# Adamtaranto/mimeo

Measured on AMD Instinct MI355X. Metric: Gbp-aligned/sec (mimeo self, 1 Gbp genome, --minIdt 80 --minLen 100 --minCov 3), higher is better.
Workload: dtype int32

## Files before the change

mimeo_amd/csrc/k6.h:

```cpp
#pragma once
#include <algorithm>
#include <cstdio>
#include <cstdlib>
#include <vector>

#include "device_util.h"

namespace mimeo {

constexpr int32_t NEG = -(1 << 30);
constexpr int32_t NEGH = -(1 << 29);

struct Cell {
    int32_t s;
    uint32_t nm, nx;
};
struct HalfResult {
    int32_t score;
    uint32_t i, j, nm, nx, overflow;
    uint32_t maxcols, rows;
    uint32_t base_lo, base_hi;
};
struct DpJob {
    uint32_t group, at, aq;
// ... 130 lines not shown
        }
        nt = dir > 0 ? min(nt, c) : max(nt, c);
    }
    for (int o = 32; o > 0; o >>= 1) {
        kmin = max(kmin, __shfl_xor(kmin, o));
        kmax = min(kmax, __shfl_xor(kmax, o));
        const long long on = __shfl_xor(nt, o);
        nt = dir > 0 ? min(nt, on) : max(nt, on);
    }
    RowBound r;
    r.kmin = wave_uniform_ll(kmin); r.kmax = wave_uniform_ll(kmax);
    nt = wave_uniform_ll(nt);
    const long long nrow = dir > 0 ? nt - (long long)at + 1 : (long long)at - nt;
    r.next = nrow > 0xFFFFFFFEll ? 0xFFFFFFFFu : (uint32_t)nrow;
    r.any = (r.kmin > -K_INF || r.kmax < K_INF) ? 1u : 0u;
    return r;
}
__device__ __forceinline__ bool bounds_none(const BoundCtx &B, uint64_t b0, uint32_t nacc, uint32_t at, int dir) {
    bool hit = false;
    for (uint32_t e = threadIdx.x & 63u; e < nacc; e += 64u) {
        const mimeo_alignment o = B.aln[b0 + e];
        if (o.tend > o.tstart && (dir > 0 ? o.tend > at : o.tstart < at)) hit = true;
    }
    return __ballot(hit) == 0;
}

struct K6Buffers {
    DeviceBuf anchors, packed, jobs, res, cnt, astate, ovf_list, any;
    DeviceBuf pidx, accrank, arena, pool, tjobs, tres, tctr;
    DeviceBuf kjobs, pcnt, pslot, ptmp;
    DeviceBuf sweep;
};
extern K6Buffers g_k6;
int dp_round(Group *d_groups, uint32_t n, const mimeo_params *p, int32_t cap, bool bounded, const BoundCtx &bc, unsigned int *novf);
int arena_reserve(uint64_t blocks, uint64_t used);
struct TraceStats { uint64_t arena_used, largest; float ms; uint32_t slices; };
int trace_round(Group *d_groups, const DpJob *d_jobs, uint32_t h0, const mimeo_params *p, int32_t cap, uint64_t budget, TraceStats &ts, bool bounded, BoundCtx bc);
int paths_pass(Group *d_groups, uint32_t ngroups, const mimeo_params *p, int32_t cap, const mimeo_alignment *d_aln, uint64_t budget, bool k6_stats);

}
```

mimeo_amd/csrc/k6_dp.hip:

```cpp
#include "k6_band.h"

namespace mimeo {

template <int WSTRIP>
__device__ __forceinline__ void load_qbits(const GStrandView &Q, uint32_t aq, int dir, uint32_t jb, uint32_t lenB,
                                           uint32_t &qlo, uint32_t &qhi, uint32_t &qn) {
    constexpr uint32_t SMASK = WSTRIP == 32 ? 0xFFFFFFFFu : ((1u << (WSTRIP & 31)) - 1u);
    if (jb > lenB) { qlo = qhi = qn = 0; return; }
    if (dir > 0) {
        int32_t p = (int32_t)(aq + jb) - 1;
        const Win32 w = win32(Q, p);
        qlo = w.lo & SMASK; qhi = w.hi & SMASK; qn = w.nm & SMASK;
    } else {
        int32_t p = (int32_t)aq - (int32_t)jb - (WSTRIP - 1);
        const Win32 w = win32(Q, p);
        qlo = __brev(w.lo & SMASK) >> (32 - WSTRIP); qhi = __brev(w.hi & SMASK) >> (32 - WSTRIP);
        qn = __brev(w.nm & SMASK) >> (32 - WSTRIP);
    }
}

struct RowBases { uint32_t lo, hi, nm; };
__device__ __forceinline__ RowBases load_row_bases(const GStrandView &T, uint32_t at, int dir, uint32_t i0) {
    if (dir > 0) {
        const Win32 w = win32(T, (int32_t)(at + i0 - 1u));
// ... 110 lines not shown
        if (rl == 63u) { best.overflow = 1; break; }
        best.maxcols = max(best.maxcols, (rl + 1u) * WSTRIP);
        best.rows = i;
        if (__ballot(rb.s > best.score)) {
            const Best4 t = wave_best(rb);
            if (t.s > best.score) { best.score = t.s; best.i = i; best.j = t.j; best.nm = t.nm; best.nx = t.nx; }
            if (best.score > cap) { best.overflow = 1; break; }
        }
        const uint32_t fmask = (uint32_t)__builtin_amdgcn_readlane((int)amask, (int)rf);
        const uint32_t plo = wb + rf * WSTRIP + (uint32_t)__builtin_ctz(fmask);
        const uint32_t nwb = plo & ~(uint32_t)(WSTRIP - 1);
        if (nwb != wb) {
            const uint32_t shift = (nwb - wb) / WSTRIP;
            wb = nwb;
            jb = wb + lane * WSTRIP;
            const int src = (int)((lane + shift) & 63u);
            const bool fresh = lane + shift >= 64u;
#pragma unroll
            for (int s = 0; s < WSTRIP; s++) {
                int32_t cs = __shfl(Cs[s], src), ds = __shfl(Ds[s], src);
                Cm[s] = __shfl(Cm[s], src); Cx[s] = __shfl(Cx[s], src);
                Dm[s] = __shfl(Dm[s], src); Dx[s] = __shfl(Dx[s], src);
                Cs[s] = fresh ? NEG : cs;
                Ds[s] = fresh ? NEG : ds;
            }
            uint32_t a0 = __shfl(qlo, src), a1 = __shfl(qhi, src), a2 = __shfl(qn, src);
            if (fresh) load_qbits<WSTRIP>(Q, aq, dir, jb, lenB, qlo, qhi, qn);
            else { qlo = a0; qhi = a1; qn = a2; }
        }
    }
    return best;
}

constexpr int L_WS = 14, L_WINDOW = 64 * L_WS;
struct LeanState {
    int32_t C[L_WS], D[L_WS];
    uint32_t Cc[L_WS], Dc[L_WS], sel[L_WS];
};
struct PCell {
    int32_t s;
    uint32_t c;
};
__device__ __forceinline__ PCell pcmax_left(const PCell &l, const PCell &r) { return r.s > l.s ? r : l; }
template <int CTRL, int RMASK>
__device__ __forceinline__ PCell dpp_pcell(const PCell &c) {
    PCell o;
    o.s = __builtin_amdgcn_update_dpp(NEG, c.s, CTRL, RMASK, 0xf, false);
    o.c = (uint32_t)__builtin_amdgcn_update_dpp(0, (int)c.c, CTRL, RMASK, 0xf, false);
    return o;
}

__device__ __forceinline__ int32_t wave_max_i32(int32_t v) {
    v = max(v, __builtin_amdgcn_update_dpp(INT32_MIN, v, 0x111, 0xf, 0xf, false));
    v = max(v, __builtin_amdgcn_update_dpp(INT32_MIN, v, 0x112, 0xf, 0xf, false));
    v = max(v, __builtin_amdgcn_update_dpp(INT32_MIN, v, 0x114, 0xf, 0xf, false));
    v = max(v, __builtin_amdgcn_update_dpp(INT32_MIN, v, 0x118, 0xf, 0xf, false));
    v = max(v, __builtin_amdgcn_update_dpp(INT32_MIN, v, 0x142, 0xa, 0xf, false));
    v = max(v, __builtin_amdgcn_update_dpp(INT32_MIN, v, 0x143, 0xc, 0xf, false));
    return __builtin_amdgcn_readlane(v, 63);
}

template <int CTRL, int RMASK>
__device__ __forceinline__ PCell lean_scan_step(const PCell &v) {
    PCell o;
    o.s = __builtin_amdgcn_update_dpp(v.s, v.s, CTRL, RMASK, 0xf, false);
    o.c = (uint32_t)__builtin_amdgcn_update_dpp((int)v.c, (int)v.c, CTRL, RMASK, 0xf, false);
    return pcmax_left(o, v);
}
__device__ __forceinline__ PCell lean_incl_maxscan(PCell v) {
    v = lean_scan_step<0x111, 0xf>(v);
    v = lean_scan_step<0x112, 0xf>(v);
    v = lean_scan_step<0x114, 0xf>(v);
    v = lean_scan_step<0x118, 0xf>(v);
    v = lean_scan_step<0x142, 0xa>(v);
    v = lean_scan_step<0x143, 0xc>(v);
    return v;
}

__device__ __forceinline__ void lean_selectors(LeanState &S, uint32_t qlo, uint32_t qhi, uint32_t qn) {
#pragma unroll
    for (int s = 0; s < L_WS; s++) {
        const uint32_t idx = ((qlo >> s) & 1u) | (((qhi >> s) & 1u) << 1);
        S.sel[s] = 0x0C0C0C00u | (((qn >> s) & 1u) ? 4u : idx);
    }
}

template <bool EDGE, bool BND = false>
__device__ __forceinline__ int32_t lean_row(LeanState &S, uint32_t srow, int32_t O, int32_t E, int32_t thr, uint32_t exmask,
                                            int32_t lane_base, int32_t kneg128) {
    const int32_t OE = O + E;
    PCell pc = dpp_pcell<0x138, 0xf>(PCell{S.C[L_WS - 1], S.Cc[L_WS - 1]});
#pragma unroll
    for (int s = L_WS - 1; s >= 0; s--) {
        const int32_t t1 = S.D[s] - E, t2 = S.C[s] - OE;
        const bool open = t2 > t1;
        const int32_t ds = max(t1, t2);
        const uint32_t dc = open ? S.Cc[s] : S.Dc[s];
        const PCell left = s ? PCell{S.C[s ? s - 1 : 0], S.Cc[s ? s - 1 : 0]} : pc;
        const uint32_t scb = __builtin_amdgcn_perm(28u, srow, S.sel[s]);
        const int32_t gs = left.s + (int32_t)scb + kneg128;
        const uint32_t gc = left.c + 0x10000u + ((int32_t)scb > 128 ? 1u : 0u);
        const bool vert = ds > gs;
        S.D[s] = ds; S.Dc[s] = dc;
        S.C[s] = max(gs, ds);
        if (BND) S.C[s] = ((exmask >> s) & 1u) ? S.C[s] : NEG;
        S.Cc[s] = vert ? dc : gc;
    }
    PCell run{NEG, 0};
#pragma unroll
    for (int s = 0; s < L_WS; s++) {
        const bool take = S.C[s] > run.s;
        run.c = take ? S.Cc[s] : run.c;
        run.s = max(run.s, S.C[s]) - E;
    }
    run.s += lane_base;
    PCell acc = dpp_pcell<0x138, 0xf>(lean_incl_maxscan(run));
    acc.s += L_WS * E - lane_base;
    int32_t rowmax = NEG;
#pragma unroll
    for (int s = 0; s < L_WS; s++) {
        const int32_t hs = S.C[s];
        const uint32_t hc = S.Cc[s];
        const int32_t is = acc.s - O;
        const bool ins = is > hs;
        const int32_t cs = max(hs, is);
        const uint32_t cc = ins ? acc.c : hc;
        const bool take = hs > acc.s;
        acc.c = take ? hc : acc.c;
        acc.s = max(acc.s, hs) - E;
        bool alive = cs >= thr;
        if (EDGE) alive = alive && ((exmask >> s) & 1u);
        S.C[s] = alive ? cs : NEG; S.Cc[s] = cc;
        S.D[s] = alive ? S.D[s] : NEG;
        rowmax = max(rowmax, S.C[s]);
    }
    return rowmax;
}

template <bool BOUND>
__device__ HalfResult wave_half_extend_lean(const GStrandView &T, const GStrandView &Q, uint32_t at, uint32_t aq, int dir,
                                            int32_t O, int32_t E, int32_t Y, const BoundCtx &B, uint64_t b0, uint32_t nacc,
                                            HalfSweep *sw) {
    const uint32_t lane = threadIdx.x & 63u;
    const uint32_t lenA = dir > 0 ? T.len - at : at, lenB = dir > 0 ? Q.len - aq : aq;
    HalfResult best{0, 0, 0, 0, 0, 0, 0, 0};
    if (BOUND) *sw = HalfSweep{0, 0, nacc, 0};
    if ((!BOUND || bounds_none(B, b0, nacc, at, dir)) && identical_suffix(T, Q, at, aq, dir, best)) return best;
    uint32_t tab[4];
#pragma unroll
    for (uint32_t a = 0; a < 4; a++) {
        uint32_t w = 0;
#pragma unroll
        for (uint32_t b = 0; b < 4; b++) {
            const uint32_t alo = a & 1u, ahi = a >> 1, dl = alo ^ (b & 1u), dh = ahi ^ (b >> 1);
            w |= (uint32_t)(sub_score(dl, dh, alo ^ ahi, 0u) + 128) << (8u * b);
        }
        tab[a] = w;
    }
    LeanState S;
    uint32_t wb = 0, jb = lane * L_WS;
    {
        uint32_t qlo, qhi, qn;
        load_qbits<L_WS>(Q, aq, dir, jb, lenB, qlo, qhi, qn);
        lean_selectors(S, qlo, qhi, qn);
    }
    bool over = false;
#pragma unroll
    for (int s = 0; s < L_WS; s++) {
        const uint32_t j = jb + s;
        const int32_t v = j ? -O - (int32_t)j * E : 0;
        const bool alive = j <= lenB && (j == 0 || v >= -Y);
        S.C[s] = alive ? v : NEG; S.Cc[s] = 0;
        S.D[s] = NEG; S.Dc[s] = 0;
        if (alive && j >= (uint32_t)(L_WINDOW - L_WS)) over = true;
    }
    if (__ballot(over)) { best.overflow = 1; return best; }
    const int32_t lane_base = (int32_t)(lane * L_WS) * E;
    const int32_t kneg128 = __builtin_amdgcn_readfirstlane(-128);
    uint32_t exmask = (1u << L_WS) - 1u;
    bool edge = wb + (uint32_t)L_WINDOW - 1u > lenB;
    if (edge) {
        exmask = 0;
#pragma unroll
        for (int s = 0; s < L_WS; s++) exmask |= (jb + s <= lenB ? 1u : 0u) << s;
    }
    long long bkmin = -K_INF, bkmax = K_INF;
    uint32_t bnext = 1u;
    int32_t klo = INT32_MAX, khi = INT32_MIN;
    RowBases rbase{0, 0, 0}, rnext = load_row_bases(T, at, dir, 1u);
    for (uint32_t i = 1; i <= lenA; i++) {
        if (i >= 0xFFFFu) { best.overflow = 1; break; }
        if (BOUND && i == bnext) {
            const RowBound rb = bounds_at(B, b0, nacc, at, aq, dir, i);
            bkmin = rb.kmin; bkmax = rb.kmax; bnext = rb.next;
        }
        const int32_t thr = best.score - Y;
        const uint32_t rbit = (i - 1u) & 31u;
        if (rbit == 0) { rbase = rnext; rnext = load_row_bases(T, at, dir, i + 32u); }
        const uint32_t rlo = (uint32_t)__builtin_amdgcn_readfirstlane((int)rbase.lo), rhi = (uint32_t)__builtin_amdgcn_readfirstlane((int)rbase.hi),
                       rnm = (uint32_t)__builtin_amdgcn_readfirstlane((int)rbase.nm);
        const uint32_t a = ((rlo >> rbit) & 1u) | (((rhi >> rbit) & 1u) << 1);
        uint32_t srow = a & 2u ? (a & 1u ? tab[3] : tab[2]) : (a & 1u ? tab[1] : tab[0]);
        if ((rnm >> rbit) & 1u) srow = 0x1C1C1C1Cu;
        uint32_t bm = 0;
        bool cut = false;
        if (BOUND) {
            const long long jlo = bkmin + (long long)i + 1, jhi = bkmax + (long long)i - 1;
            if (bkmin > -K_INF || bkmax < K_INF) sw->nbound++;
            cut = jlo > (long long)wb || jhi < (long long)wb + (L_WINDOW - 1);
            const long long r0 = jlo - (long long)jb, r1 = jhi - (long long)jb + 1;
            const uint32_t s0 = (uint32_t)min(max(r0, 0ll), (long long)L_WS), s1 = (uint32_t)min(max(r1, 0ll), (long long)L_WS);
            bm = ((1u << s1) - 1u) & ~((1u << s0) - 1u) & exmask;
        }
        const int32_t rowmax = BOUND && cut ? lean_row<true, true>(S, srow, O, E, thr, bm, lane_base, kneg128)
                               : edge ? lean_row<true>(S, srow, O, E, thr, exmask, lane_base, kneg128)
                                      : lean_row<false>(S, srow, O, E, thr, exmask, lane_base, kneg128);
        const uint64_t ball = __ballot(rowmax > NEGH);
        if (!ball) break;
        const uint32_t rf = (uint32_t)__builtin_ctzll(ball), rl = 63u - (uint32_t)__builtin_clzll(ball);
        if (rl == 63u) { best.overflow = 1; break; }
        best.maxcols = max(best.maxcols, (rl + 1u) * L_WS);
        best.rows = i;
        if (BOUND) {
            klo = min(klo, (int32_t)((long long)wb + rf * L_WS - (long long)i));
            khi = max(khi, (int32_t)((long long)wb + (rl + 1u) * L_WS - 1 - (long long)i));
        }
        const int32_t wmax = wave_max_i32(rowmax);
        if (wmax > best.score) {
            const uint32_t L = (uint32_t)__builtin_ctzll(__ballot(rowmax == wmax));
            uint32_t slot = 0, cnt = 0;
#pragma unroll
            for (int s = L_WS - 1; s >= 0; s--) {
                const int32_t v = __builtin_amdgcn_readlane(S.C[s], (int)L);
                if (v == wmax) { slot = (uint32_t)s; cnt = (uint32_t)__builtin_amdgcn_readlane((int)S.Cc[s], (int)L); }
            }
            best.score = wmax; best.i = i; best.j = wb + L * L_WS + slot; best.nm = cnt & 0xFFFFu; best.nx = (cnt >> 16) - (cnt & 0xFFFFu);
        }
        if (rf) {
            wb += rf * L_WS;
            jb = wb + lane * L_WS;
            const int src = (int)((lane + rf) & 63u);
            const bool fresh = lane + rf >= 64u;
#pragma unroll
            for (int s = 0; s < L_WS; s++) {
                const int32_t cs = __shfl(S.C[s], src), ds = __shfl(S.D[s], src);
                S.Cc[s] = __shfl(S.Cc[s], src); S.Dc[s] = __shfl(S.Dc[s], src);
                S.sel[s] = __shfl(S.sel[s], src);
                S.C[s] = fresh ? NEG : cs;
                S.D[s] = fresh ? NEG : ds;
            }
            if (fresh) {
                uint32_t qlo, qhi, qn;
                load_qbits<L_WS>(Q, aq, dir, jb, lenB, qlo, qhi, qn);
                lean_selectors(S, qlo, qhi, qn);
            }
            edge = wb + (uint32_t)L_WINDOW - 1u > lenB;
            if (edge) {
                exmask = 0;
#pragma unroll
                for (int s = 0; s < L_WS; s++) exmask |= (jb + s <= lenB ? 1u : 0u) << s;
            } else if (BOUND) exmask = (1u << L_WS) - 1u;
        }
    }
    if (BOUND) { sw->klo = klo; sw->khi = khi; }
    return best;
}

__global__ __launch_bounds__(64) void k6_dp1(const Group *__restrict__ groups, const DpJob *__restrict__ jobs,
                                             HalfResult *__restrict__ res, int32_t O, int32_t E, int32_t Y) {
    const DpJob job = jobs[blockIdx.x];
    const Group &G = groups[job.group];
    HalfResult r = wave_half_extend_lean<false>(G.T, G.Q, job.at, job.aq, job.dir, O, E, Y, BoundCtx{}, 0, 0, nullptr);
    if (threadIdx.x == 0) res[job.slot] = r;
}

__global__ __launch_bounds__(64) void k6_dp1_bounded(const Group *__restrict__ groups, const DpJob *__restrict__ jobs,
                                                     HalfResult *__restrict__ res, HalfSweep *__restrict__ sweep, int32_t O, int32_t E,
                                                     int32_t Y, BoundCtx B, unsigned int *__restrict__ novf,
                                                     unsigned int *__restrict__ ovf_list) {
    const DpJob job = jobs[blockIdx.x];
    const Group &G = groups[job.group];
    HalfSweep sw;
    HalfResult r = wave_half_extend_lean<true>(G.T, G.Q, job.at, job.aq, job.dir, O, E, Y, B, G.hsp_begin, G.nacc, &sw);
    if (threadIdx.x == 0) {
        res[job.slot] = r;
        sweep[job.slot] = sw;
        if (r.overflow) ovf_list[atomicAdd(novf, 1u)] = blockIdx.x;
    }
}

__global__ __launch_bounds__(64) void k6_dp_wide(const Group *__restrict__ groups, const DpJob *__restrict__ jobs,
                                                 HalfResult *__restrict__ res, int32_t O, int32_t E, int32_t Y,
                                                 unsigned int *__restrict__ novf, unsigned int *__restrict__ ovf_list, int32_t cap,
                                                 int every) {
    const DpJob job = jobs[blockIdx.x];
    if (!every && !res[job.slot].overflow) return;
    const Group &G = groups[job.group];
    HalfResult r = wave_half_extend_2048(G.T, G.Q, job.at, job.aq, job.dir, O, E, Y, cap);
    if (threadIdx.x == 0) {
        res[job.slot] = r;
        if (r.overflow) ovf_list[atomicAdd(novf, 1u)] = blockIdx.x;
    }
}

constexpr uint32_t ANY_COLS = 1u << 16;
constexpr int ANY_THREADS = 1024;
struct AnyRow {
    int32_t *cs, *ds;
    uint32_t *cm, *cx, *dm, *dx;
};
__device__ __forceinline__ AnyRow any_row(uint32_t *base, uint32_t parity) {
    uint32_t *b = base + (size_t)parity * 6u * ANY_COLS;
    return AnyRow{(int32_t *)b, (int32_t *)(b + ANY_COLS), b + 2u * ANY_COLS, b + 3u * ANY_COLS, b + 4u * ANY_COLS, b + 5u * ANY_COLS};
}
constexpr size_t ANY_SLOT_WORDS = 2u * 6u * (size_t)ANY_COLS;

// ... 17 lines not shown
        if (diag) { g.nm = P.cm[(j - 1) & M] + (m ? 1u : 0u); g.nx = P.cx[(j - 1) & M] + (m ? 0u : 1u); }
        N.dm[j & M] = dd.nm; N.dx[j & M] = dd.nx;
        const Cell hh = hd ? dd : g;
        N.cm[j & M] = hh.nm; N.cx[j & M] = hh.nx;
        return hh;
    }
    __device__ __forceinline__ Cell htag(uint32_t j) const { return Cell{0, N.cm[j & M], N.cx[j & M]}; }
    __device__ __forceinline__ Cell c(uint32_t j, const Cell &ht, const Cell &ia, bool ci) const { const Cell ct = ci ? ia : ht; N.cm[j & M] = ct.nm; N.cx[j & M] = ct.nx; return ct; }
};

template <bool BOUND>
__global__ __launch_bounds__(ANY_THREADS) void k6_dp_any(const Group *__restrict__ groups, const DpJob *__restrict__ jobs,
                                                         const unsigned int *__restrict__ list, uint32_t first,
                                                         HalfResult *__restrict__ res, uint32_t *__restrict__ scratch,
                                                         int32_t O, int32_t E, int32_t Y, int32_t cap, BoundCtx B,
                                                         HalfSweep *__restrict__ sweep) {
    const DpJob job = jobs[list[first + blockIdx.x]];
    const Group &G = groups[job.group];
    const uint32_t lenA = job.dir > 0 ? G.T.len - job.at : job.at;
    CountRows rows{scratch + (size_t)blockIdx.x * ANY_SLOT_WORDS};
    HalfSweep sw;
    const HalfResult r = band_dp<ANY_THREADS, BOUND>(rows, G, job, lenA, O, E, Y, cap, B, sw);
    if (threadIdx.x == 0) res[job.slot] = r;
    if (BOUND && threadIdx.x == 0) sweep[job.slot] = sw;
}

__global__ void k6_list_all(uint32_t n, unsigned int *__restrict__ novf, unsigned int *__restrict__ ovf_list) {
    const uint32_t k = blockIdx.x * blockDim.x + threadIdx.x;
    if (k < n) ovf_list[k] = k;
    if (k == 0) *novf = n;
}

int dp_round(Group *d_groups, uint32_t n, const mimeo_params *p, int32_t cap, bool bounded, const BoundCtx &bc,
                    unsigned int *novf) {
    hipStream_t st = stream();
    int rc;
    const Group *groups = d_groups;
    const DpJob *jobs = (const DpJob *)g_k6.jobs.p;
    HalfResult *res = (HalfResult *)g_k6.res.p;
    HalfSweep *sweep = bounded ? (HalfSweep *)g_k6.sweep.p : nullptr;
    unsigned int *list = (unsigned int *)g_k6.ovf_list.p;
    const int32_t O = p->gap_open, E = p->gap_extend, Y = p->ydrop;
    const bool lean_ok = E <= (1 << 16) && O <= (1 << 24) && Y <= (1 << 28);
    if (bounded) {
        if (lean_ok) hipLaunchKernelGGL(k6_dp1_bounded, dim3(n), dim3(64), 0, st, groups, jobs, res, sweep, O, E, Y, bc, novf, list);
        else hipLaunchKernelGGL(k6_list_all, dim3((n + 255) / 256), dim3(256), 0, st, n, novf, list);
    } else {
        if (lean_ok) hipLaunchKernelGGL(k6_dp1, dim3(n), dim3(64), 0, st, groups, jobs, res, O, E, Y);
        hipLaunchKernelGGL(k6_dp_wide, dim3(n), dim3(64), 0, st, groups, jobs, res, O, E, Y, novf, list, cap, lean_ok ? 0 : 1);
    }
    unsigned int nov = 0;
    HIP_TRY(hipMemcpyAsync(&nov, novf, 4, hipMemcpyDeviceToHost, st));
    HIP_TRY(hipStreamSynchronize(st));
    if (!nov) return 0;
    const unsigned int slots = std::min<unsigned int>(nov, 32u);
    if ((rc = g_k6.any.reserve((size_t)slots * ANY_SLOT_WORDS * 4))) return rc;
    const auto any = bounded ? k6_dp_any<true> : k6_dp_any<false>;
    for (unsigned int f = 0; f < nov; f += slots)
        hipLaunchKernelGGL(any, dim3(std::min(slots, nov - f)), dim3(ANY_THREADS), 0, st, groups, jobs, (const unsigned int *)list, f, res,
                           (uint32_t *)g_k6.any.p, O, E, Y, cap, bc, sweep);
    return 0;
}

}
```

mimeo_amd/csrc/k6_gapped.hip:

```cpp
#include "k6.h"

namespace mimeo {

constexpr uint32_t ANCHOR_W = 31, ANCHOR_CHUNK = 4096;
constexpr int ANCHOR_THREADS = 1024;

__device__ void wave_anchor_chunk(const GStrandView &T, const GStrandView &Q, const mimeo_hsp &h, uint32_t chunk,
                                  unsigned long long *packed) {
    const uint32_t lane = threadIdx.x & 63u, nw = h.length - ANCHOR_W + 1;
    const int32_t d = (int32_t)h.tstart - (int32_t)h.qstart;
    const uint32_t w0 = chunk * ANCHOR_CHUNK + lane * (ANCHOR_CHUNK / 64u), w1 = min(nw, w0 + ANCHOR_CHUNK / 64u);
    int32_t bs = INT32_MIN;
    uint32_t bw = 0xFFFFFFFFu;
    if (w0 < w1) {
        int32_t sum = 0;
        bool m;
        for (uint32_t k = 0; k < ANCHOR_W; k++) {
            int32_t pt = (int32_t)(h.tstart + w0 + k);
            sum += pair_score(T, Q, pt, pt - d, &m);
        }
        bs = sum; bw = w0;
        for (uint32_t w = w0 + 1; w < w1; w++) {
            int32_t add = (int32_t)(h.tstart + w + ANCHOR_W - 1), sub = (int32_t)(h.tstart + w - 1);
            sum += pair_score(T, Q, add, add - d, &m) - pair_score(T, Q, sub, sub - d, &m);
// ... 303 lines not shown

__global__ void k6_kept_ranks(Group *__restrict__ groups, uint32_t ngroups, const mimeo_alignment *__restrict__ aln,
                              uint32_t *__restrict__ accrank, const uint2 *__restrict__ pidx, int32_t thresh) {
    const uint32_t g = blockIdx.x * blockDim.x + threadIdx.x;
    if (g >= ngroups) return;
    Group &G = groups[g];
    const uint64_t b0 = G.hsp_begin;
    uint32_t k = 0;
    for (uint32_t e = 0; e < G.nacc; e++) {
        if (aln[b0 + e].score < thresh) continue;
        const uint32_t rank = accrank[b0 + e];
        const uint32_t slot = 2u * (uint32_t)(b0 + rank);
        if (pidx[slot].x == PATH_UNTRACED || pidx[slot + 1].x == PATH_UNTRACED) G.overflow = 1;
        accrank[b0 + k++] = rank;
    }
}

__global__ __launch_bounds__(256) void k6_ungapped_paths(const Group *__restrict__ groups, const mimeo_alignment *__restrict__ aln,
                                                         PathBlock *__restrict__ arena, uint2 *__restrict__ pidx,
                                                         uint32_t *__restrict__ accrank) {
    const Group &G = groups[blockIdx.x];
    const uint64_t b0 = G.hsp_begin;
    for (uint32_t r = threadIdx.x; r < G.nacc; r += 256) {
        const mimeo_alignment a = aln[b0 + r];
        arena[b0 + r] = PathBlock{a.tstart, a.qstart, a.tend - a.tstart};
        pidx[2u * (b0 + r)] = make_uint2((uint32_t)(b0 + r), 1u);
        pidx[2u * (b0 + r) + 1u] = make_uint2(0u, 0u);
        accrank[b0 + r] = r;
    }
}

K6Buffers g_k6;

static int round_stats(uint32_t n, uint64_t nhsps, bool bounded, unsigned long long *bound_jobs) {
    std::vector<DpJob> hj(n);
    std::vector<HalfResult> hall((size_t)nhsps * 2), hr(n);
    HIP_TRY(hipStreamSynchronize(stream()));
    HIP_TRY(hipMemcpy(hj.data(), g_k6.jobs.p, (size_t)n * sizeof(DpJob), hipMemcpyDeviceToHost));
    HIP_TRY(hipMemcpy(hall.data(), g_k6.res.p, hall.size() * sizeof(HalfResult), hipMemcpyDeviceToHost));
    for (size_t k = 0; k < hr.size(); k++) hr[k] = hall[hj[k].slot];
    unsigned long long hist[9] = {0}, rows = 0, maxr = 0, shortcut = 0;
    for (auto &r : hr) {
        if (!r.rows) { shortcut++; continue; }
        hist[std::min<uint32_t>(8, r.maxcols / 128)]++; rows += r.rows; maxr = std::max<unsigned long long>(maxr, r.rows);
    }
    unsigned long long rebased = 0;
    for (auto &r : hr) if (r.base_lo | r.base_hi) rebased++;
    fprintf(stderr, "[k6] jobs %u shortcut %llu (rebased in k6_dp_any: %llu) rows total %llu max %llu band<128..>=1024:", n, shortcut, rebased, rows, maxr);
    for (int b = 0; b < 9; b++) fprintf(stderr, " %llu", hist[b]);
    fprintf(stderr, "\n");
    {
        unsigned long long fine[34] = {0};
        for (auto &r : hr) if (r.rows) fine[std::min<uint32_t>(33, r.maxcols / 32)]++;
        fprintf(stderr, "[k6] widest band, buckets of 32 columns from 448:");
        for (int b = 14; b < 34; b++) fprintf(stderr, " %llu", fine[b]);
        fprintf(stderr, "\n");
    }
    if (n <= 8)
        for (size_t k = 0; k < hr.size(); k++)
            fprintf(stderr, "  [k6] job %zu: dir %d rows %u maxcols %u i %u j %u rebased %d\n", k, hj[k].dir, hr[k].rows, hr[k].maxcols, hr[k].i, hr[k].j,
                    (hr[k].base_lo | hr[k].base_hi) ? 1 : 0);
    int shown = 0;
    for (auto &r : hr)
        if (!r.rows && shown < 8) { fprintf(stderr, "  [k6] zero-row job: score %d i %u j %u nm %u nx %u ovf %u\n", r.score, r.i, r.j, r.nm, r.nx, r.overflow); shown++; }
    if (bounded) {
        std::vector<HalfSweep> hs((size_t)nhsps * 2);
        HIP_TRY(hipMemcpy(hs.data(), g_k6.sweep.p, hs.size() * sizeof(HalfSweep), hipMemcpyDeviceToHost));
        for (auto &j : hj) *bound_jobs += hs[j.slot].nbound ? 1u : 0u;
    }
    return 0;
}

struct K6Call {
    uint32_t bmax, rounds;
    bool stats, path, bounded, box_paths;
    int32_t cap;
    uint64_t pool_budget;
    unsigned long long bound_jobs, rescheduled;
    TraceStats ts;
};

static int gapped_setup(Group *d_groups, uint32_t ngroups, const mimeo_hsp *d_sorted, const uint32_t *d_order, uint64_t nhsps, K6Call &c) {
    c.bmax = getenv("MIMEO_K6_BMAX") ? (uint32_t)atoi(getenv("MIMEO_K6_BMAX")) : 8192u / ngroups;
    c.bmax = c.bmax < 1 ? 1 : (c.bmax > MAX_BATCH ? MAX_BATCH : c.bmax);
    c.stats = getenv("MIMEO_K6_STATS") != nullptr;
    c.cap = getenv("MIMEO_K6_SCORE_CAP") ? std::max(100000, atoi(getenv("MIMEO_K6_SCORE_CAP"))) : 2000000000;
    hipStream_t st = stream();
    int rc;
    if ((rc = g_k6.anchors.reserve(nhsps * sizeof(uint2)))) return rc;
    if ((rc = g_k6.packed.reserve(nhsps * 8))) return rc;
    HIP_TRY(hipMemsetAsync(g_k6.packed.p, 0, nhsps * 8, st));
    if ((rc = g_k6.jobs.reserve((size_t)ngroups * c.bmax * 2 * sizeof(DpJob)))) return rc;
    if ((rc = g_k6.res.reserve((size_t)nhsps * 2 * sizeof(HalfResult)))) return rc;
    if ((rc = g_k6.astate.reserve((size_t)nhsps * 2))) return rc;
    HIP_TRY(hipMemsetAsync(g_k6.astate.p, 0, (size_t)nhsps * 2, st));
    if ((rc = g_k6.cnt.reserve(16))) return rc;
    if ((rc = g_k6.ovf_list.reserve((size_t)ngroups * c.bmax * 2 * sizeof(unsigned int)))) return rc;
    const uint32_t asplit = ngroups > 4096 ? 1u : ANCHOR_SPLIT;
    hipLaunchKernelGGL(k6_anchor_points, dim3(ngroups, asplit), dim3(ANCHOR_THREADS), 0, st, (const Group *)d_groups,
                       d_sorted, d_order, (unsigned long long *)g_k6.packed.p);
    hipLaunchKernelGGL(k6_anchor_final, dim3(ngroups), dim3(256), 0, st, (const Group *)d_groups, d_sorted, d_order,
                       (const unsigned long long *)g_k6.packed.p, (uint2 *)g_k6.anchors.p);
    if (c.path || c.box_paths) {
        if ((rc = g_k6.tctr.reserve(16))) return rc;
        if ((rc = arena_reserve(1024, 0))) return rc;
        HIP_TRY(hipMemsetAsync(g_k6.tctr.p, 0, 16, st));
        size_t free_b = 0, total_b = 0;
        HIP_TRY(hipMemGetInfo(&free_b, &total_b));
        c.pool_budget = std::min<uint64_t>(((uint64_t)free_b + g_k6.pool.cap) / 4, 16ull << 30);
        if (getenv("MIMEO_K6_TRACE_POOL_MB")) c.pool_budget = (uint64_t)atol(getenv("MIMEO_K6_TRACE_POOL_MB")) << 20;
    }
    if (c.bounded && (rc = g_k6.sweep.reserve((size_t)nhsps * 2 * sizeof(HalfSweep)))) return rc;
    return 0;
}

static int gapped_rounds(Group *d_groups, uint32_t ngroups, uint64_t nhsps, const mimeo_params *p, mimeo_alignment *d_aln, K6Call &c) {
    hipStream_t st = stream();
    int rc;
    PathView pv{nullptr, nullptr, nullptr};
    if (c.path || c.box_paths) pv = PathView{(const uint2 *)g_k6.pidx.p, nullptr, (uint32_t *)g_k6.accrank.p};
    const auto pick = c.path ? k6_pick<true> : k6_pick<false>;
    const auto resolve = c.bounded ? k6_resolve<true, true> : c.path ? k6_resolve<true, false>
                         : c.box_paths ? k6_resolve<false, false, true> : k6_resolve<false, false>;
    const HalfSweep *sweep = c.bounded ? (const HalfSweep *)g_k6.sweep.p : nullptr;
    for (;;) {
        HIP_TRY(hipMemsetAsync(g_k6.cnt.p, 0, 16, st));
        unsigned int *njobs = (unsigned int *)g_k6.cnt.p, *remaining = njobs + 1, *novf = njobs + 2;
        pv.blk = (const PathBlock *)g_k6.arena.p;
        hipLaunchKernelGGL(pick, dim3(ngroups), dim3(64), 0, st, d_groups, (const uint2 *)g_k6.anchors.p, (const mimeo_alignment *)d_aln,
                           c.bmax, (uint8_t *)g_k6.astate.p, (uint8_t *)g_k6.astate.p + nhsps, (DpJob *)g_k6.jobs.p, njobs, pv);
        unsigned int h0 = 0;
        HIP_TRY(hipMemcpyAsync(&h0, njobs, 4, hipMemcpyDeviceToHost, st));
        HIP_TRY(hipStreamSynchronize(st));
        if (h0) {
            const BoundCtx bc{(const mimeo_alignment *)d_aln, (const uint2 *)g_k6.anchors.p, pv};
            if ((rc = dp_round(d_groups, h0, p, c.cap, c.bounded, bc, novf))) return rc;
            if (c.stats && (rc = round_stats(h0, nhsps, c.bounded, &c.bound_jobs))) return rc;
            if (c.path) {
                c.rounds++;
                if ((rc = trace_round(d_groups, (const DpJob *)g_k6.jobs.p, h0, p, c.cap, c.pool_budget, c.ts, c.bounded, bc))) return rc;
                pv.blk = (const PathBlock *)g_k6.arena.p;
            }
        }
        hipLaunchKernelGGL(resolve, dim3(ngroups), dim3(64), 0, st, d_groups, (const uint2 *)g_k6.anchors.p, (const HalfResult *)g_k6.res.p,
                           d_aln, (uint8_t *)g_k6.astate.p, remaining, pv, sweep);
        unsigned int h4[4] = {0, 0, 0, 0};
        HIP_TRY(hipMemcpyAsync(h4, g_k6.cnt.p, 16, hipMemcpyDeviceToHost, st));
        HIP_TRY(hipStreamSynchronize(st));
        c.rescheduled += h4[3];
        if (!h4[1]) return 0;
    }
}

static void path_rule_stats(const K6Call &c) {
    fprintf(stderr, "[k6] path rule: traceback %.3f ms, rounds %u slices %u, %llu path blocks, pool %.1f MB, largest half %.3f MB", c.ts.ms,
            c.rounds, c.ts.slices, (unsigned long long)c.ts.arena_used, g_k6.pool.cap / 1048576.0, c.ts.largest / 1048576.0);
    if (c.bounded) fprintf(stderr, ", bounded jobs %llu, rescheduled %llu", c.bound_jobs, c.rescheduled);
    fprintf(stderr, "\n");
}

int gapped_device(Group *d_groups, uint32_t ngroups, const mimeo_hsp *d_sorted, const uint32_t *d_order,
                  uint64_t nhsps, const mimeo_params *p, mimeo_alignment *d_aln, bool want_paths) {
    if (!ngroups || !nhsps) return 0;
    hipStream_t st = stream();
    int rc;
    const bool path = p->gapped && p->anchor_rule == MIMEO_ANCHOR_PATH;
    if (want_paths && nhsps >= (1ull << 31)) { set_error("paths: more than 2^31 HSPs in one batch"); return MIMEO_ERR_LIMIT; }
    if (want_paths || path) {
        if ((rc = g_k6.pidx.reserve((size_t)nhsps * 2 * sizeof(uint2)))) return rc;
        if ((rc = g_k6.accrank.reserve((size_t)nhsps * 4))) return rc;
// ... 26 lines not shown
```

Before: 0.04868.

## Run unbounded lean DP at half strip width, widening state on band overflow

The unbounded lean DP now starts with 7 columns per lane, giving a 448-column window instead of 896, which cuts per-lane register state. When the band reaches the second-to-last lane, the wave repacks its state into the 14-column layout and continues from that row. If the narrow start overflows at row 0 or on the band edge, the wave restarts at full width. Restart and widen counters are added for the stats path. The aim is lower register pressure and less per-row work for the many narrow jobs, at the cost of an extra code path and redundant work when a job has to restart.

Measured after the change: 0.05033, median of 6. 3.4% higher.

```diff
diff --git a/mimeo_amd/csrc/k6.h b/mimeo_amd/csrc/k6.h
--- a/mimeo_amd/csrc/k6.h
+++ b/mimeo_amd/csrc/k6.h
@@ -186,7 +186,7 @@
     DeviceBuf sweep;
 };
 extern K6Buffers g_k6;
-int dp_round(Group *d_groups, uint32_t n, const mimeo_params *p, int32_t cap, bool bounded, const BoundCtx &bc, unsigned int *novf);
+int dp_round(Group *d_groups, uint32_t n, const mimeo_params *p, int32_t cap, bool bounded, const BoundCtx &bc, unsigned int *novf, unsigned int *nrestart);
 int arena_reserve(uint64_t blocks, uint64_t used);
 struct TraceStats { uint64_t arena_used, largest; float ms; uint32_t slices; };
 int trace_round(Group *d_groups, const DpJob *d_jobs, uint32_t h0, const mimeo_params *p, int32_t cap, uint64_t budget, TraceStats &ts, bool bounded, BoundCtx bc);
diff --git a/mimeo_amd/csrc/k6_dp.hip b/mimeo_amd/csrc/k6_dp.hip
--- a/mimeo_amd/csrc/k6_dp.hip
+++ b/mimeo_amd/csrc/k6_dp.hip
@@ -166,10 +166,19 @@
     return best;
 }
 
-constexpr int L_WS = 14, L_WINDOW = 64 * L_WS;
+constexpr int L_WS = 14;
+constexpr int L_W1 = 7;
+static_assert(2 * L_W1 == L_WS, "lean_widen pairs up strips of L_W1 columns, and maxcols is counted in whole strips of L_WS");
+constexpr uint32_t LEAN_BAND = 1u, LEAN_ROWS = 2u, LEAN_WIDEN = 3u;
+struct ScoreTab { uint32_t t0, t1, t2, t3; };
+template <int WS>
 struct LeanState {
-    int32_t C[L_WS], D[L_WS];
-    uint32_t Cc[L_WS], Dc[L_WS], sel[L_WS];
+    int32_t C[WS], D[WS];
+    uint32_t Cc[WS], Dc[WS], sel[WS];
+};
+struct LeanHandover {
+    HalfResult best;
+    uint32_t rows, wb;
 };
 struct PCell {
     int32_t s;
@@ -211,21 +220,22 @@
     return v;
 }
 
-__device__ __forceinline__ void lean_selectors(LeanState &S, uint32_t qlo, uint32_t qhi, uint32_t qn) {
-#pragma unroll
-    for (int s = 0; s < L_WS; s++) {
+template <int WS>
+__device__ __forceinline__ void lean_selectors(LeanState<WS> &S, uint32_t qlo, uint32_t qhi, uint32_t qn) {
+#pragma unroll
+    for (int s = 0; s < WS; s++) {
         const uint32_t idx = ((qlo >> s) & 1u) | (((qhi >> s) & 1u) << 1);
         S.sel[s] = 0x0C0C0C00u | (((qn >> s) & 1u) ? 4u : idx);
     }
 }
 
-template <bool EDGE, bool BND = false>
-__device__ __forceinline__ int32_t lean_row(LeanState &S, uint32_t srow, int32_t O, int32_t E, int32_t thr, uint32_t exmask,
+template <int WS, bool EDGE, bool BND = false>
+__device__ __forceinline__ int32_t lean_row(LeanState<WS> &S, uint32_t srow, int32_t O, int32_t E, int32_t thr, uint32_t exmask,
                                             int32_t lane_base, int32_t kneg128) {
     const int32_t OE = O + E;
-    PCell pc = dpp_pcell<0x138, 0xf>(PCell{S.C[L_WS - 1], S.Cc[L_WS - 1]});
-#pragma unroll
-    for (int s = L_WS - 1; s >= 0; s--) {
+    PCell pc = dpp_pcell<0x138, 0xf>(PCell{S.C[WS - 1], S.Cc[WS - 1]});
+#pragma unroll
+    for (int s = WS - 1; s >= 0; s--) {
         const int32_t t1 = S.D[s] - E, t2 = S.C[s] - OE;
         const bool open = t2 > t1;
         const int32_t ds = max(t1, t2);
@@ -242,17 +252,17 @@
     }
     PCell run{NEG, 0};
 #pragma unroll
-    for (int s = 0; s < L_WS; s++) {
+    for (int s = 0; s < WS; s++) {
         const bool take = S.C[s] > run.s;
         run.c = take ? S.Cc[s] : run.c;
         run.s = max(run.s, S.C[s]) - E;
     }
     run.s += lane_base;
     PCell acc = dpp_pcell<0x138, 0xf>(lean_incl_maxscan(run));
-    acc.s += L_WS * E - lane_base;
+    acc.s += WS * E - lane_base;
     int32_t rowmax = NEG;
 #pragma unroll
-    for (int s = 0; s < L_WS; s++) {
+    for (int s = 0; s < WS; s++) {
         const int32_t hs = S.C[s];
         const uint32_t hc = S.Cc[s];
         const int32_t is = acc.s - O;
@@ -271,59 +281,56 @@
     return rowmax;
 }
 
-template <bool BOUND>
-__device__ HalfResult wave_half_extend_lean(const GStrandView &T, const GStrandView &Q, uint32_t at, uint32_t aq, int dir,
-                                            int32_t O, int32_t E, int32_t Y, const BoundCtx &B, uint64_t b0, uint32_t nacc,
-                                            HalfSweep *sw) {
-    const uint32_t lane = threadIdx.x & 63u;
-    const uint32_t lenA = dir > 0 ? T.len - at : at, lenB = dir > 0 ? Q.len - aq : aq;
-    HalfResult best{0, 0, 0, 0, 0, 0, 0, 0};
-    if (BOUND) *sw = HalfSweep{0, 0, nacc, 0};
-    if ((!BOUND || bounds_none(B, b0, nacc, at, dir)) && identical_suffix(T, Q, at, aq, dir, best)) return best;
-    uint32_t tab[4];
-#pragma unroll
-    for (uint32_t a = 0; a < 4; a++) {
-        uint32_t w = 0;
-#pragma unroll
-        for (uint32_t b = 0; b < 4; b++) {
-            const uint32_t alo = a & 1u, ahi = a >> 1, dl = alo ^ (b & 1u), dh = ahi ^ (b >> 1);
-            w |= (uint32_t)(sub_score(dl, dh, alo ^ ahi, 0u) + 128) << (8u * b);
-        }
-        tab[a] = w;
-    }
-    LeanState S;
-    uint32_t wb = 0, jb = lane * L_WS;
-    {
-        uint32_t qlo, qhi, qn;
-        load_qbits<L_WS>(Q, aq, dir, jb, lenB, qlo, qhi, qn);
-        lean_selectors(S, qlo, qhi, qn);
-    }
+template <int WS>
+__device__ __forceinline__ bool lean_row0(const GStrandView &Q, uint32_t aq, int dir, uint32_t lenB, int32_t O, int32_t E, int32_t Y,
+                                          LeanState<WS> &S) {
+    const uint32_t jb = (threadIdx.x & 63u) * WS;
+    uint32_t qlo, qhi, qn;
+    load_qbits<WS>(Q, aq, dir, jb, lenB, qlo, qhi, qn);
+    lean_selectors<WS>(S, qlo, qhi, qn);
     bool over = false;
 #pragma unroll
-    for (int s = 0; s < L_WS; s++) {
+    for (int s = 0; s < WS; s++) {
         const uint32_t j = jb + s;
         const int32_t v = j ? -O - (int32_t)j * E : 0;
         const bool alive = j <= lenB && (j == 0 || v >= -Y);
         S.C[s] = alive ? v : NEG; S.Cc[s] = 0;
         S.D[s] = NEG; S.Dc[s] = 0;
-        if (alive && j >= (uint32_t)(L_WINDOW - L_WS)) over = true;
-    }
-    if (__ballot(over)) { best.overflow = 1; return best; }
-    const int32_t lane_base = (int32_t)(lane * L_WS) * E;
+        if (alive && j >= (uint32_t)(64 * WS - WS)) over = true;
+    }
+    return __ballot(over) == 0;
+}
+
+template <int WS, bool BOUND>
+__device__ __forceinline__ HalfResult lean_dp(const GStrandView &T, const GStrandView &Q, uint32_t at, uint32_t aq, int dir, int32_t O,
+                                              int32_t E, int32_t Y, const ScoreTab tab, const BoundCtx &B, uint64_t b0, uint32_t nacc,
+                                              HalfSweep *sw, LeanState<WS> &S, LeanHandover &ho) {
+    static_assert(!BOUND || WS == L_WS, "the bounded kernel runs at the full width");
+    constexpr int WINDOW = 64 * WS;
+    constexpr bool WIDENS = WS == L_W1;
+    const uint32_t lane = threadIdx.x & 63u;
+    const uint32_t lenA = dir > 0 ? T.len - at : at, lenB = dir > 0 ? Q.len - aq : aq;
+    HalfResult best = ho.best;
+    best.overflow = 0;
+    uint32_t wb = ho.wb, jb = wb + lane * WS;
+    const uint32_t i0 = ho.rows + 1u;
+    const int32_t lane_base = (int32_t)(lane * WS) * E;
     const int32_t kneg128 = __builtin_amdgcn_readfirstlane(-128);
-    uint32_t exmask = (1u << L_WS) - 1u;
-    bool edge = wb + (uint32_t)L_WINDOW - 1u > lenB;
+    uint32_t exmask = (1u << WS) - 1u;
+    bool edge = wb + (uint32_t)WINDOW - 1u > lenB;
     if (edge) {
         exmask = 0;
 #pragma unroll
-        for (int s = 0; s < L_WS; s++) exmask |= (jb + s <= lenB ? 1u : 0u) << s;
+        for (int s = 0; s < WS; s++) exmask |= (jb + s <= lenB ? 1u : 0u) << s;
     }
     long long bkmin = -K_INF, bkmax = K_INF;
     uint32_t bnext = 1u;
     int32_t klo = INT32_MAX, khi = INT32_MIN;
-    RowBases rbase{0, 0, 0}, rnext = load_row_bases(T, at, dir, 1u);
-    for (uint32_t i = 1; i <= lenA; i++) {
-        if (i >= 0xFFFFu) { best.overflow = 1; break; }
+    const uint32_t blk = ((i0 - 1u) & ~31u) + 1u;
+    RowBases rbase{0, 0, 0}, rnext = load_row_bases(T, at, dir, blk);
+    if ((i0 - 1u) & 31u) { rbase = rnext; rnext = load_row_bases(T, at, dir, blk + 32u); }
+    for (uint32_t i = i0; i <= lenA; i++) {
+        if (i >= 0xFFFFu) { best.overflow = LEAN_ROWS; break; }
         if (BOUND && i == bnext) {
             const RowBound rb = bounds_at(B, b0, nacc, at, aq, dir, i);
             bkmin = rb.kmin; bkmax = rb.kmax; bnext = rb.next;
@@ -334,49 +341,53 @@
         const uint32_t rlo = (uint32_t)__builtin_amdgcn_readfirstlane((int)rbase.lo), rhi = (uint32_t)__builtin_amdgcn_readfirstlane((int)rbase.hi),
                        rnm = (uint32_t)__builtin_amdgcn_readfirstlane((int)rbase.nm);
         const uint32_t a = ((rlo >> rbit) & 1u) | (((rhi >> rbit) & 1u) << 1);
-        uint32_t srow = a & 2u ? (a & 1u ? tab[3] : tab[2]) : (a & 1u ? tab[1] : tab[0]);
+        uint32_t srow = a & 2u ? (a & 1u ? tab.t3 : tab.t2) : (a & 1u ? tab.t1 : tab.t0);
         if ((rnm >> rbit) & 1u) srow = 0x1C1C1C1Cu;
         uint32_t bm = 0;
         bool cut = false;
         if (BOUND) {
             const long long jlo = bkmin + (long long)i + 1, jhi = bkmax + (long long)i - 1;
             if (bkmin > -K_INF || bkmax < K_INF) sw->nbound++;
-            cut = jlo > (long long)wb || jhi < (long long)wb + (L_WINDOW - 1);
+            cut = jlo > (long long)wb || jhi < (long long)wb + (WINDOW - 1);
             const long long r0 = jlo - (long long)jb, r1 = jhi - (long long)jb + 1;
-            const uint32_t s0 = (uint32_t)min(max(r0, 0ll), (long long)L_WS), s1 = (uint32_t)min(max(r1, 0ll), (long long)L_WS);
+            const uint32_t s0 = (uint32_t)min(max(r0, 0ll), (long long)WS), s1 = (uint32_t)min(max(r1, 0ll), (long long)WS);
             bm = ((1u << s1) - 1u) & ~((1u << s0) - 1u) & exmask;
         }
-        const int32_t rowmax = BOUND && cut ? lean_row<true, true>(S, srow, O, E, thr, bm, lane_base, kneg128)
-                               : edge ? lean_row<true>(S, srow, O, E, thr, exmask, lane_base, kneg128)
-                                      : lean_row<false>(S, srow, O, E, thr, exmask, lane_base, kneg128);
+        const int32_t rowmax = BOUND && cut ? lean_row<WS, true, true>(S, srow, O, E, thr, bm, lane_base, kneg128)
+                               : edge ? lean_row<WS, true>(S, srow, O, E, thr, exmask, lane_base, kneg128)
+                                      : lean_row<WS, false>(S, srow, O, E, thr, exmask, lane_base, kneg128);
         const uint64_t ball = __ballot(rowmax > NEGH);
         if (!ball) break;
         const uint32_t rf = (uint32_t)__builtin_ctzll(ball), rl = 63u - (uint32_t)__builtin_clzll(ball);
-        if (rl == 63u) { best.overflow = 1; break; }
-        best.maxcols = max(best.maxcols, (rl + 1u) * L_WS);
+        if (rl == 63u) { best.overflow = LEAN_BAND; break; }
+        if constexpr (WS == L_WS) {
+            best.maxcols = max(best.maxcols, (rl + 1u) * WS);
+        } else {
+            best.maxcols = max(best.maxcols, ((wb + rl * WS) / L_WS + 1u - wb / L_WS) * L_WS);
+        }
         best.rows = i;
         if (BOUND) {
-            klo = min(klo, (int32_t)((long long)wb + rf * L_WS - (long long)i));
-            khi = max(khi, (int32_t)((long long)wb + (rl + 1u) * L_WS - 1 - (long long)i));
+            klo = min(klo, (int32_t)((long long)wb + rf * WS - (long long)i));
+            khi = max(khi, (int32_t)((long long)wb + (rl + 1u) * WS - 1 - (long long)i));
         }
         const int32_t wmax = wave_max_i32(rowmax);
         if (wmax > best.score) {
             const uint32_t L = (uint32_t)__builtin_ctzll(__ballot(rowmax == wmax));
             uint32_t slot = 0, cnt = 0;
 #pragma unroll
-            for (int s = L_WS - 1; s >= 0; s--) {
+            for (int s = WS - 1; s >= 0; s--) {
                 const int32_t v = __builtin_amdgcn_readlane(S.C[s], (int)L);
                 if (v == wmax) { slot = (uint32_t)s; cnt = (uint32_t)__builtin_amdgcn_readlane((int)S.Cc[s], (int)L); }
             }
-            best.score = wmax; best.i = i; best.j = wb + L * L_WS + slot; best.nm = cnt & 0xFFFFu; best.nx = (cnt >> 16) - (cnt & 0xFFFFu);
+            best.score = wmax; best.i = i; best.j = wb + L * WS + slot; best.nm = cnt & 0xFFFFu; best.nx = (cnt >> 16) - (cnt & 0xFFFFu);
         }
         if (rf) {
-            wb += rf * L_WS;
-            jb = wb + lane * L_WS;
+            wb += rf * WS;
+            jb = wb + lane * WS;
             const int src = (int)((lane + rf) & 63u);
             const bool fresh = lane + rf >= 64u;
 #pragma unroll
-            for (int s = 0; s < L_WS; s++) {
+            for (int s = 0; s < WS; s++) {
                 const int32_t cs = __shfl(S.C[s], src), ds = __shfl(S.D[s], src);
                 S.Cc[s] = __shfl(S.Cc[s], src); S.Dc[s] = __shfl(S.Dc[s], src);
                 S.sel[s] = __shfl(S.sel[s], src);
@@ -385,27 +396,99 @@
             }
             if (fresh) {
                 uint32_t qlo, qhi, qn;
-                load_qbits<L_WS>(Q, aq, dir, jb, lenB, qlo, qhi, qn);
-                lean_selectors(S, qlo, qhi, qn);
+                load_qbits<WS>(Q, aq, dir, jb, lenB, qlo, qhi, qn);
+                lean_selectors<WS>(S, qlo, qhi, qn);
             }
-            edge = wb + (uint32_t)L_WINDOW - 1u > lenB;
+            edge = wb + (uint32_t)WINDOW - 1u > lenB;
             if (edge) {
                 exmask = 0;
 #pragma unroll
-                for (int s = 0; s < L_WS; s++) exmask |= (jb + s <= lenB ? 1u : 0u) << s;
-            } else if (BOUND) exmask = (1u << L_WS) - 1u;
-        }
+                for (int s = 0; s < WS; s++) exmask |= (jb + s <= lenB ? 1u : 0u) << s;
+            } else if (BOUND) exmask = (1u << WS) - 1u;
+        }
+        if (WIDENS && rl == 62u) { best.overflow = LEAN_WIDEN; ho.best = best; ho.rows = i; ho.wb = wb; break; }
     }
     if (BOUND) { sw->klo = klo; sw->khi = khi; }
     return best;
 }
 
+__device__ __forceinline__ void lean_widen(const LeanState<L_W1> &N, LeanState<L_WS> &S, uint32_t &wb, const GStrandView &Q, uint32_t aq,
+                                           int dir, uint32_t lenB) {
+    const uint32_t lane = threadIdx.x & 63u;
+    const int odd = (int)((wb / L_W1) & 1u);
+    wb -= (uint32_t)odd * L_W1;
+#pragma unroll
+    for (int h = 0; h < 2; h++) {
+        const int src = 2 * (int)lane + h - odd;
+        const bool dead = src < 0 || src > 63;
+#pragma unroll
+        for (int s = 0; s < L_W1; s++) {
+            const int32_t cs = __shfl(N.C[s], src & 63), ds = __shfl(N.D[s], src & 63);
+            S.Cc[h * L_W1 + s] = __shfl(N.Cc[s], src & 63); S.Dc[h * L_W1 + s] = __shfl(N.Dc[s], src & 63);
+            S.C[h * L_W1 + s] = dead ? NEG : cs;
+            S.D[h * L_W1 + s] = dead ? NEG : ds;
+        }
+    }
+    uint32_t qlo, qhi, qn;
+    load_qbits<L_WS>(Q, aq, dir, wb + lane * L_WS, lenB, qlo, qhi, qn);
+    lean_selectors<L_WS>(S, qlo, qhi, qn);
+}
+
+template <bool BOUND>
+__device__ HalfResult wave_half_extend_lean(const GStrandView &T, const GStrandView &Q, uint32_t at, uint32_t aq, int dir,
+                                            int32_t O, int32_t E, int32_t Y, const BoundCtx &B, uint64_t b0, uint32_t nacc,
+                                            HalfSweep *sw, uint32_t *event) {
+    HalfResult best{0, 0, 0, 0, 0, 0, 0, 0};
+    if (BOUND) *sw = HalfSweep{0, 0, nacc, 0};
+    if ((!BOUND || bounds_none(B, b0, nacc, at, dir)) && identical_suffix(T, Q, at, aq, dir, best)) return best;
+    uint32_t t[4];
+#pragma unroll
+    for (uint32_t a = 0; a < 4; a++) {
+        uint32_t w = 0;
+#pragma unroll
+        for (uint32_t b = 0; b < 4; b++) {
+            const uint32_t alo = a & 1u, ahi = a >> 1, dl = alo ^ (b & 1u), dh = ahi ^ (b >> 1);
+            w |= (uint32_t)(sub_score(dl, dh, alo ^ ahi, 0u) + 128) << (8u * b);
+        }
+        t[a] = w;
+    }
+    const ScoreTab tab{t[0], t[1], t[2], t[3]};
+    const uint32_t lenB = dir > 0 ? Q.len - aq : aq;
+    LeanState<L_WS> S;
+    LeanHandover ho{best, 0u, 0u};
+    bool full0 = true;
+    if constexpr (!BOUND) {
+        LeanState<L_W1> N;
+        if (lean_row0<L_W1>(Q, aq, dir, lenB, O, E, Y, N)) {
+            best = lean_dp<L_W1, false>(T, Q, at, aq, dir, O, E, Y, tab, B, b0, nacc, sw, N, ho);
+            if (best.overflow == 0u || best.overflow == LEAN_ROWS) { best.overflow = best.overflow ? 1u : 0u; return best; }
+        } else best.overflow = LEAN_BAND;
+        if (best.overflow == LEAN_WIDEN) {
+            lean_widen(N, S, ho.wb, Q, aq, dir, lenB);
+            full0 = false;
+            *event = LEAN_WIDEN;
+        } else {
+            ho = LeanHandover{HalfResult{0, 0, 0, 0, 0, 0, 0, 0}, 0u, 0u};
+            *event = LEAN_BAND;
+        }
+    }
+    if (full0 && !lean_row0<L_WS>(Q, aq, dir, lenB, O, E, Y, S)) { best = HalfResult{0, 0, 0, 0, 0, 0, 0, 0}; best.overflow = 1u; return best; }
+    best = lean_dp<L_WS, BOUND>(T, Q, at, aq, dir, O, E, Y, tab, B, b0, nacc, sw, S, ho);
+    best.overflow = best.overflow ? 1u : 0u;
+    return best;
+}
+
 __global__ __launch_bounds__(64) void k6_dp1(const Group *__restrict__ groups, const DpJob *__restrict__ jobs,
-                                             HalfResult *__restrict__ res, int32_t O, int32_t E, int32_t Y) {
+                                             HalfResult *__restrict__ res, int32_t O, int32_t E, int32_t Y,
+                                             unsigned int *__restrict__ nrestart) {
     const DpJob job = jobs[blockIdx.x];
     const Group &G = groups[job.group];
-    HalfResult r = wave_half_extend_lean<false>(G.T, G.Q, job.at, job.aq, job.dir, O, E, Y, BoundCtx{}, 0, 0, nullptr);
-    if (threadIdx.x == 0) res[job.slot] = r;
+    uint32_t event = 0;
+    HalfResult r = wave_half_extend_lean<false>(G.T, G.Q, job.at, job.aq, job.dir, O, E, Y, BoundCtx{}, 0, 0, nullptr, &event);
+    if (threadIdx.x == 0) {
+        res[job.slot] = r;
+        if (event) atomicAdd(nrestart + (event == LEAN_WIDEN ? 1 : 0), 1u);
+    }
 }
 
 __global__ __launch_bounds__(64) void k6_dp1_bounded(const Group *__restrict__ groups, const DpJob *__restrict__ jobs,
@@ -415,7 +498,7 @@
     const DpJob job = jobs[blockIdx.x];
     const Group &G = groups[job.group];
     HalfSweep sw;
-    HalfResult r = wave_half_extend_lean<true>(G.T, G.Q, job.at, job.aq, job.dir, O, E, Y, B, G.hsp_begin, G.nacc, &sw);
+    HalfResult r = wave_half_extend_lean<true>(G.T, G.Q, job.at, job.aq, job.dir, O, E, Y, B, G.hsp_begin, G.nacc, &sw, nullptr);
     if (threadIdx.x == 0) {
         res[job.slot] = r;
         sweep[job.slot] = sw;
@@ -499,7 +582,7 @@
 }
 
 int dp_round(Group *d_groups, uint32_t n, const mimeo_params *p, int32_t cap, bool bounded, const BoundCtx &bc,
-                    unsigned int *novf) {
+                    unsigned int *novf, unsigned int *nrestart) {
     hipStream_t st = stream();
     int rc;
     const Group *groups = d_groups;
@@ -513,7 +596,7 @@
         if (lean_ok) hipLaunchKernelGGL(k6_dp1_bounded, dim3(n), dim3(64), 0, st, groups, jobs, res, sweep, O, E, Y, bc, novf, list);
         else hipLaunchKernelGGL(k6_list_all, dim3((n + 255) / 256), dim3(256), 0, st, n, novf, list);
     } else {
-        if (lean_ok) hipLaunchKernelGGL(k6_dp1, dim3(n), dim3(64), 0, st, groups, jobs, res, O, E, Y);
+        if (lean_ok) hipLaunchKernelGGL(k6_dp1, dim3(n), dim3(64), 0, st, groups, jobs, res, O, E, Y, nrestart);
         hipLaunchKernelGGL(k6_dp_wide, dim3(n), dim3(64), 0, st, groups, jobs, res, O, E, Y, novf, list, cap, lean_ok ? 0 : 1);
     }
     unsigned int nov = 0;
diff --git a/mimeo_amd/csrc/k6_gapped.hip b/mimeo_amd/csrc/k6_gapped.hip
--- a/mimeo_amd/csrc/k6_gapped.hip
+++ b/mimeo_amd/csrc/k6_gapped.hip
@@ -359,7 +359,7 @@
 
 K6Buffers g_k6;
 
-static int round_stats(uint32_t n, uint64_t nhsps, bool bounded, unsigned long long *bound_jobs) {
+static int round_stats(uint32_t n, uint64_t nhsps, bool bounded, unsigned long long *bound_jobs, const unsigned int *nrestart) {
     std::vector<DpJob> hj(n);
     std::vector<HalfResult> hall((size_t)nhsps * 2), hr(n);
     HIP_TRY(hipStreamSynchronize(stream()));
@@ -373,6 +373,9 @@
     }
     unsigned long long rebased = 0;
     for (auto &r : hr) if (r.base_lo | r.base_hi) rebased++;
+    unsigned int wide[2] = {0, 0};
+    HIP_TRY(hipMemcpy(wide, nrestart, 8, hipMemcpyDeviceToHost));
+    fprintf(stderr, "[k6] full strip width: restarted %u widened %u of %u\n", wide[0], wide[1], n);
     fprintf(stderr, "[k6] jobs %u shortcut %llu (rebased in k6_dp_any: %llu) rows total %llu max %llu band<128..>=1024:", n, shortcut, rebased, rows, maxr);
     for (int b = 0; b < 9; b++) fprintf(stderr, " %llu", hist[b]);
     fprintf(stderr, "\n");
@@ -421,7 +424,7 @@
     if ((rc = g_k6.res.reserve((size_t)nhsps * 2 * sizeof(HalfResult)))) return rc;
     if ((rc = g_k6.astate.reserve((size_t)nhsps * 2))) return rc;
     HIP_TRY(hipMemsetAsync(g_k6.astate.p, 0, (size_t)nhsps * 2, st));
-    if ((rc = g_k6.cnt.reserve(16))) return rc;
+    if ((rc = g_k6.cnt.reserve(32))) return rc;
     if ((rc = g_k6.ovf_list.reserve((size_t)ngroups * c.bmax * 2 * sizeof(unsigned int)))) return rc;
     const uint32_t asplit = ngroups > 4096 ? 1u : ANCHOR_SPLIT;
     hipLaunchKernelGGL(k6_anchor_points, dim3(ngroups, asplit), dim3(ANCHOR_THREADS), 0, st, (const Group *)d_groups,
@@ -451,8 +454,8 @@
                          : c.box_paths ? k6_resolve<false, false, true> : k6_resolve<false, false>;
     const HalfSweep *sweep = c.bounded ? (const HalfSweep *)g_k6.sweep.p : nullptr;
     for (;;) {
-        HIP_TRY(hipMemsetAsync(g_k6.cnt.p, 0, 16, st));
-        unsigned int *njobs = (unsigned int *)g_k6.cnt.p, *remaining = njobs + 1, *novf = njobs + 2;
+        HIP_TRY(hipMemsetAsync(g_k6.cnt.p, 0, 32, st));
+        unsigned int *njobs = (unsigned int *)g_k6.cnt.p, *remaining = njobs + 1, *novf = njobs + 2, *nrestart = njobs + 4;
         pv.blk = (const PathBlock *)g_k6.arena.p;
         hipLaunchKernelGGL(pick, dim3(ngroups), dim3(64), 0, st, d_groups, (const uint2 *)g_k6.anchors.p, (const mimeo_alignment *)d_aln,
                            c.bmax, (uint8_t *)g_k6.astate.p, (uint8_t *)g_k6.astate.p + nhsps, (DpJob *)g_k6.jobs.p, njobs, pv);
@@ -461,8 +464,8 @@
         HIP_TRY(hipStreamSynchronize(st));
         if (h0) {
             const BoundCtx bc{(const mimeo_alignment *)d_aln, (const uint2 *)g_k6.anchors.p, pv};
-            if ((rc = dp_round(d_groups, h0, p, c.cap, c.bounded, bc, novf))) return rc;
-            if (c.stats && (rc = round_stats(h0, nhsps, c.bounded, &c.bound_jobs))) return rc;
+            if ((rc = dp_round(d_groups, h0, p, c.cap, c.bounded, bc, novf, nrestart))) return rc;
+            if (c.stats && (rc = round_stats(h0, nhsps, c.bounded, &c.bound_jobs, nrestart))) return rc;
             if (c.path) {
                 c.rounds++;
                 if ((rc = trace_round(d_groups, (const DpJob *)g_k6.jobs.p, h0, p, c.cap, c.pool_budget, c.ts, c.bounded, bc))) return rc;
```
